# lunarlab-gatech/SLIDE_SLAM

Hardware: AMD Instinct MI355X
Metric: pose-graph updates/sec + ms/Gauss-Newton iter, 8-robot 10k-landmark graph (higher is better)
Workload: dtype f64

## Files before the change

slide_slam_amd/csrc/chol_kernels.hip:

```cpp
#include <hip/hip_runtime.h>
#include <stdlib.h>
#include <algorithm>
#include <type_traits>
#include <utility>
#include <vector>

#include "graph_dev.hpp"
#include "kernels.hpp"

namespace sl {

typedef double v4d __attribute__((ext_vector_type(4)));
constexpr int CHOL_BATCH_MAX = 8;
__device__ inline v4d mfma_f64(double a, double b, v4d c) { return __builtin_amdgcn_mfma_f64_16x16x4f64(a, b, c, 0, 0, 0); }

__device__ inline double rsqrt_nr(double d) {
#ifdef SLIDE_RSQRT_OLD
  double y = __builtin_amdgcn_rsq(d);
  y = y * (1.5 - 0.5 * d * y * y);
  y = y * (1.5 - 0.5 * d * y * y);
  return y;
#else
  double y = __builtin_amdgcn_rsq(d);
  double t = d * y, h = 0.5 * y;
// ... 2551 lines not shown
    const int ka = std::max(1, ks_sys ? ks_sys[0] : ks), kb = std::max(1, ks_sys ? ks_sys[1] : ks), km = std::max(ka, kb);
    A.ks = km; A.scratch = scratch; A.scratch_stride = std::max<size_t>(1, (size_t)(nb + 1) * nb * (km - 1) * NB * NB);
    A.ks_sys[0] = ka; A.ks_sys[1] = kb;
    launch_syrk_kernel(dim3(njobs, 1, km), lds_pad, s, A);
    hipLaunchKernelGGL(k_border_syrk_reduce2, dim3(16 * (nb + 1), jb_end >= 0 ? jb_end : nb), dim3(256), 0, s, d[0].bord, d[0].ldb, d[1].bord, d[1].ldb, nb,
                       ka, kb, scratch, scratch + A.scratch_stride, d[0].T, d[1].T);
    return;
  }
  if (scratch && n == 1 && ks > 1) {
    A.ks = ks; A.scratch = scratch;
    launch_syrk_kernel(dim3(njobs, 1, ks), lds_pad, s, A);
    const int nb = d[0].nbr;
    hipLaunchKernelGGL(k_border_syrk_reduce, dim3(16 * (nb + 1), jb_end >= 0 ? jb_end : nb), dim3(256), 0, s, d[0].bord, d[0].ldb, nb, ks, scratch, d[0].bfirst, d[0].T);
    return;
  }
  launch_syrk_kernel(dim3(njobs), lds_pad, s, A);
}
struct BorderApplyArgs {
  int n;
  const double* S[CHOL_BATCH_MAX]; int ld[CHOL_BATCH_MAX]; int T[CHOL_BATCH_MAX]; int nbr[CHOL_BATCH_MAX]; int b0[CHOL_BATCH_MAX];
  double* yv[CHOL_BATCH_MAX]; const double* x[CHOL_BATCH_MAX];
  const int* segtab[CHOL_BATCH_MAX];
};
__global__ __launch_bounds__(256) void k_border_apply(BorderApplyArgs A) {
  const int r = blockIdx.z;
  const int col = blockIdx.x * 4 + (threadIdx.x >> 6), lane = threadIdx.x & 63;
  if (col >= A.T[r] * NB) return;
  const int nrow = A.nbr[r] * NB;
  const double* w = A.S[r] + (size_t)col * A.ld[r] + (size_t)A.b0[r] * NB;
  const double* x = A.x[r];
  double acc = 0.0;
  const int* st = A.segtab[r];
  const int* msk = st ? st + 1 + st[0] + st[0] * (A.nbr[r] + 1) : nullptr;
  if (msk && msk[0] > 0) {
    const int c = col / NB;
    unsigned long long m = (unsigned long long)(unsigned)msk[1 + 2 * c] | ((unsigned long long)(unsigned)msk[2 + 2 * c] << 32);
    while (m) {
      const int t = __ffsll((long long)m) - 1;
      m &= m - 1;
      acc += w[t * NB + lane] * x[t * NB + lane];
    }
  } else {
    for (int q = lane; q < nrow; q += 64) acc += w[q] * x[q];
  }
#pragma unroll
  for (int m = 32; m >= 1; m >>= 1) acc += __shfl_xor(acc, m);
  if (lane == 0) A.yv[r][col] -= acc;
}
void launch_border_apply(const CholSystem* d, int n, const double* const* xloc, hipStream_t s) {
  BorderApplyArgs A{};
  A.n = n;
  int Tmax = 0;
  for (int i = 0; i < n; ++i) {
    A.S[i] = d[i].S; A.ld[i] = d[i].ld; A.T[i] = d[i].T; A.nbr[i] = d[i].nbr; A.yv[i] = d[i].yv; A.x[i] = xloc[i];
    A.b0[i] = d[i].b0 > 0 ? d[i].b0 : d[i].T;
    A.segtab[i] = d[i].segtab;
    Tmax = d[i].T > Tmax ? d[i].T : Tmax;
  }
  if (Tmax > 0) hipLaunchKernelGGL(k_border_apply, dim3(Tmax * NB / 4, 1, n), dim3(256), 0, s, A);
}

void launch_chol_bwd_all(const double* S, int ld, int T, const double* Ld, const double* Winv, double* yv, double* dp,
                         int* status, const int* prof, hipStream_t s, const double* wf_prev, double wf_thr, int wf_Tprev, int wf_lim);
void launch_chol_extract_y(const double* S, int ld, int T, double* yv, double* dp, int* status, hipStream_t s, int nbr, int b0, double* prev) {
  hipLaunchKernelGGL(k_chol_extract_y, dim3((T * NB + 255) / 256), dim3(256), 0, s, S, ld, T, (b0 > 0 ? b0 : T) + nbr, yv, dp, status, prev);
}
struct StepPlan { int kb, nP, g0, g1, nX, TvA, TvB, TvX, nbA, nbB, nbX; long long nA, nB; };
static int chol_n_cu() {
  static int n_cu = 0;
  if (!n_cu) {
    int dev = 0;
    hipDeviceProp_t pr;
    if (hipGetDevice(&dev) == hipSuccess && hipGetDeviceProperties(&pr, dev) == hipSuccess) n_cu = pr.multiProcessorCount;
    if (n_cu <= 0) n_cu = 256;
  }
  return n_cu;
}
static StepPlan plan_step(int k, int T, const int* prof, int nbr = 0, const int* bfirst = nullptr, int kofs = 0) {
  static const double frac = getenv("SLIDE_CHOL_FRAC") ? atof(getenv("SLIDE_CHOL_FRAC")) : 0.5;
  StepPlan p{};
  p.kb = k & ~1;
  p.TvA = p.TvB = p.TvX = T;
// ... 77 lines not shown
    for (int i = 0; i < n; ++i) {
      const PairPlan p = plan_pair(k, d[i].T, d[i].h_prof, d[i].nbr, d[i].h_bfirst, d[i].kofs);
      A.S[i] = d[i].S; A.ld[i] = d[i].ld; A.Ld[i] = d[i].Ld; A.Winv[i] = d[i].Winv; A.status[i] = d[i].status;
      A.ncols[i] = p.ncols; A.Tv0[i] = p.Tv0; A.Tv1[i] = p.Tv1; A.nb0[i] = p.nb0; A.nb1[i] = p.nb1;
      A.TvB[i] = p.TvB; A.nbB[i] = p.nbB; A.nP[i] = p.nP;
      A.nbr[i] = d[i].nbr; A.B0[i] = d[i].b0 > 0 ? d[i].b0 : d[i].T; A.ord[i] = d[i].ord;
      A.a_base[i + 1] = A.a_base[i] + (int)(2 * p.nA);
      A.b_base[i + 1] = A.b_base[i] + (int)p.nB;
    }
    const long long nAw = A.a_base[n], nB = A.b_base[n];
    if (nAw <= 0) continue;
    const long long extra = nB < n_cu ? nB : n_cu;
    const long long free_cu = n_cu - nAw > 8 ? n_cu - nAw : 8;
    const int a_joins = nB > free_cu ? 1 : 0;
    hipLaunchKernelGGL(k_chol_pair_batched, dim3((unsigned)(nAw + extra)), dim3(PAIR_THREADS), 0, s, A, k, ctr, tickets, a_joins);
  }
}
bool chol_pair_supported(const CholSystem* d, int n) {
  if (n < 1 || n > CHOL_STEP_BATCH_MAX) return false;
  for (int i = 0; i < n; ++i)
    if (d[i].L32) return false;
  return true;
}
void launch_chol_batch(const CholSystem* d, int n, int* ctr, hipStream_t s, hipEvent_t after_steps, bool solve, int cu_share, int* pair_tickets) {
  const bool pair = pair_tickets != nullptr;
  const int n_cu = chol_n_cu();
  int Tmax = 0;
  for (int i = 0; i < n; ++i) Tmax = d[i].T > Tmax ? d[i].T : Tmax;
  static const bool verify = getenv("SLIDE_PAIR_VERIFY") && getenv("SLIDE_PAIR_VERIFY")[0] == '1';
  if (pair && chol_pair_supported(d, n) && verify) {
    (void)hipStreamSynchronize(s);
    std::vector<CholSystem> cp(d, d + n);
    std::vector<size_t> len(n);
    std::vector<void*> tmp;
    auto dmal = [&](size_t bytes) { void* p = nullptr; (void)hipMalloc(&p, bytes); tmp.push_back(p); return p; };
    for (int i = 0; i < n; ++i) {
      const int B0 = d[i].b0 > 0 ? d[i].b0 : d[i].T;
      len[i] = (size_t)d[i].ld * ((size_t)d[i].T * NB - 1) + (size_t)(B0 + d[i].nbr + 1) * NB;
      cp[i].S = (double*)dmal(len[i] * sizeof(double));
      cp[i].Ld = (double*)dmal((size_t)d[i].T * NB * NB * sizeof(double));
      cp[i].Winv = (double*)dmal((size_t)d[i].T * 1024 * sizeof(double));
      cp[i].status = (int*)dmal(8 * sizeof(int));
      cp[i].yv = (double*)dmal((size_t)d[i].T * NB * sizeof(double));
      cp[i].dp = (double*)dmal((size_t)d[i].T * NB * sizeof(double));
      (void)hipMemset(cp[i].status, 0, 8 * sizeof(int));
      (void)hipMemcpy(cp[i].S, d[i].S, len[i] * sizeof(double), hipMemcpyDeviceToDevice);
    }
// ... 43 lines not shown
    const int a_split = (k > 0 && (nA2 + nBt) * 100 <= (long long)n_cu * share) ? 1 : 0;
    A.a_base[0] = A.b_base[0] = 0;
    for (int i = 0; i < n; ++i) {
      A.S[i] = d[i].S; A.ld[i] = d[i].ld; A.T[i] = d[i].T; A.Ld[i] = d[i].Ld; A.Winv[i] = d[i].Winv; A.status[i] = d[i].status;
      A.L32[i] = d[i].L32;
      A.TvA[i] = pl[i].TvA; A.TvB[i] = pl[i].TvB; A.TvX[i] = pl[i].TvX;
      A.nP[i] = pl[i].nP; A.g0[i] = pl[i].g0; A.g1[i] = pl[i].g1; A.nX[i] = pl[i].nX; A.a_split[i] = a_split;
      A.nbr[i] = d[i].nbr; A.nbA[i] = pl[i].nbA; A.nbB[i] = pl[i].nbB; A.nbX[i] = pl[i].nbX;
      A.B0[i] = d[i].b0 > 0 ? d[i].b0 : d[i].T;
      A.ord[i] = d[i].ord;
      A.a_base[i + 1] = A.a_base[i] + (int)(pl[i].nA << a_split);
      A.b_base[i + 1] = A.b_base[i] + (int)pl[i].nB;
    }
    const long long nAw = A.a_base[n], nB = A.b_base[n];
    const long long extra = nB < n_cu ? nB : n_cu;
    const long long free_cu = n_cu - nAw > 8 ? n_cu - nAw : 8;
    const int a_joins = nB > free_cu ? 1 : 0;
    static const int xcd_map = getenv("SLIDE_CHOL_XCD") ? atoi(getenv("SLIDE_CHOL_XCD")) : 0;
    hipLaunchKernelGGL(k_chol_step_batched, dim3((unsigned)(nAw + extra)), dim3(512), 0, s, A, k, k & ~1, ctr, a_joins, (xcd_map && n > 1) ? 1 : 0);
  }
  if (Tmax < 0) Tmax = -Tmax;
  if (after_steps) (void)hipEventRecord(after_steps, s);
  if (!solve) {
    ExtractArgs E{};
    E.n = n;
    for (int i = 0; i < n; ++i) {
      E.S[i] = d[i].S; E.ld[i] = d[i].ld; E.T[i] = d[i].T; E.Tr[i] = (d[i].b0 > 0 ? d[i].b0 : d[i].T) + d[i].nbr;
      E.yv[i] = d[i].yv; E.dp[i] = d[i].dp; E.status[i] = d[i].status;
    }
    if (Tmax > 0) hipLaunchKernelGGL(k_chol_extract_y_b, dim3((Tmax * NB + 255) / 256, n), dim3(256), 0, s, E);
    return;
  }
  launch_chain_tables(d, n, s);
  const double* yin[CHOL_BATCH_MAX];
  double* xout[CHOL_BATCH_MAX];
  for (int i = 0; i < n; ++i) {
    launch_chol_extract_y(d[i].S, d[i].ld, d[i].T, d[i].yv, d[i].dp, d[i].status, s, d[i].nbr);
    yin[i] = d[i].yv; xout[i] = d[i].dp;
  }
  if (chain_has_tables(d, n)) {
    launch_chain_batch(d, n, yin, xout, false, false, true, nullptr, s);
    return;
  }
  launch_chol_bwd_batch(d, n, s);
}
void launch_chol_bwd_batch(const CholSystem* d, int n, hipStream_t s) {
// ... 197 lines not shown
```

slide_slam_amd/csrc/host_graph.hip:

```cpp
#include <chrono>

#include "host_graph.hpp"

#include <algorithm>
#include <cmath>
#include <cstdio>
#include <cstdlib>
#include <map>
#include <unordered_map>

namespace sl {

static inline int lam_ks_cap(int nl) {
  const int tiles = (nl + 1) * nl;
  if (tiles <= 0) return 1;
  return tiles <= 32 ? 16 : std::max(1, std::min(16, 256 / tiles));
}

thread_local std::string g_last_error;
void thread_capture_mode_local() {
  thread_local bool done = false;
  if (done) return;
  hipStreamCaptureMode m = hipStreamCaptureModeThreadLocal;
  (void)hipThreadExchangeStreamCaptureMode(&m);
// ... 1047 lines not shown
  if (whole || part == 0) {
    if (!whole) launch_bcast(d_bufs, n, 12 * ng, master);
    launch_ghost_exchange_batched(d_Gs, n, ng, 1, d_bufs, master);
  }
  return SLIDE_OK;
}
int CholBatch::enqueue_arrow(double* const* d_bufs, int part, hipEvent_t e0, hipEvent_t e1) {
  const bool whole = part < 0;
  if (part == 20) return enqueue_ghost_refresh(d_bufs, part);
  auto mark = [&](int i) { if (prof_ev[0]) (void)hipEventRecord(prof_ev[i], master); };
  const int* maps[CHOL_BATCH_HOST_MAX];
  double* xloc[CHOL_BATCH_HOST_MAX];
  for (int i = 0; i < n; ++i) { maps[i] = graphs[i]->d_sep_map.d; xloc[i] = graphs[i]->d_xloc.d; }
  const int ld_s = (sep_Ts + sep_nl + 1) * NB;
  const SepLayout Y = sep_layout();
  CholSystem lv[2];
  const int sTa = sep_leafT[0], sTL = sTa + sep_leafT[1], sTt = sep_Ts - sTL;
  if (sep_dissected()) sep_leaf_systems(lv);
  const bool owned = !whole && sep_dissected() && sep_owner >= 0;
  const int own = owned ? sep_owner : 0, own_t0 = own ? sTa : 0, own_T = sep_leafT[own];
  CholSystem top{};
  top.S = sepS + (owned ? (size_t)own_t0 * NB * ld_s : 0); top.ld = ld_s; top.T = owned ? own_T : sTL; top.b0 = sTL; top.nbr = sTt + sep_nl;
  top.bord = sepS + (size_t)sTL * NB * ld_s + (size_t)sTL * NB; top.ldb = ld_s;
  if (part == 1) {
    if (!owned) return SLIDE_OK;
    if (sep_leader) launch_sep_unpack(Y, master, sTL, sep_Ts + sep_nl);
    launch_sep_unpack(Y, master, own_t0, own_t0 + own_T);
    if (ll_leaf_own[own]) launch_chol_ll(ll_leaf_own[own], &lv[own], 1, master);
    else launch_chol_batch(&lv[own], 1, sep_ctr2, master, nullptr, false, 100, (chol_pair_mask() & 4) ? pair_tickets(10) : nullptr);
    if (sep_leader) {
      launch_border_syrk_jobs(&top, 1, d_sep_jobs, n_sep_jobs, 0, master, sep_scratch, sep_ks, sTt);
      if (sep_nl > 0) {
        CholSystem sl{};
        sl.S = sepS + (size_t)own_t0 * NB * ld_s; sl.ld = ld_s; sl.T = own_T; sl.b0 = sep_Ts; sl.nbr = sep_nl; sl.bord = sep_bord; sl.ldb = (sep_nl + 1) * NB;
        const int ks = std::max(1, std::min(lam_ks_cap(sep_nl), own_T / 2));
        launch_border_syrk(&sl, 1, master, lam_scratch, ks);
      }
      launch_sep_unpack(Y, master, sTL, sep_Ts + sep_nl, true);
    }
    return SLIDE_OK;
  }
  if (whole || part == 0) {
    launch_status_clear(d_Gs, n, master, sep_status, sep_nl > 0 ? lam_status : nullptr);
    const int rg = enqueue_ghost_refresh(d_bufs, part);
    if (rg != SLIDE_OK) return rg;
    launch_phase0_batched(d_Gs, hG.data(), n, d_bufs, master, false, rb.on() ? d_Rs : nullptr, ol.on() ? d_Os : nullptr);
    launch_phase3_arrow_batched(d_Gs, hG.data(), n, master);
    {
      int nq[CHOL_BATCH_HOST_MAX];
      for (int i = 0; i < n; ++i) nq[i] = graphs[i]->n_sep_poses;
      launch_sep_extract_batched(d_Gs, hG.data(), n, nq, master);
    }
    if (e0) (void)hipEventRecord(e0, master);
    mark(0);
    if (ll_seg) {
      launch_chol_ll(ll_seg, seg_sys.data(), (int)seg_sys.size(), master);
      last_groups = 1;
      if (e1) (void)hipEventRecord(e1, master);
    } else {
      const int rc = factor_all(e1);
      if (rc != SLIDE_OK) return rc;
    }
    mark(1);
    if (n_syrk_jobs > 0) launch_border_syrk_jobs(sys.data(), n, d_syrk_jobs, n_syrk_jobs, syrk_lds_pad, master);
    else launch_border_syrk(sys.data(), n, master);
    mark(6);
    if (!l2_sys.empty()) {
      if (ll_l2) launch_chol_ll(ll_l2, l2_sys.data(), (int)l2_sys.size(), master);
      else launch_chol_batch(l2_sys.data(), (int)l2_sys.size(), d_ctr2, master, nullptr, false, 100, (chol_pair_mask() & 2) ? pair_tickets(8) : nullptr);
      if (n_l2_jobs > 0) launch_border_syrk_jobs(l2_sys.data(), (int)l2_sys.size(), d_l2_jobs, n_l2_jobs, 0, master);
      else launch_border_syrk(l2_sys.data(), (int)l2_sys.size(), master);
    }
    mark(2);
    static const bool env_canon = !(getenv("SLIDE_SEP_CANONICAL") && getenv("SLIDE_SEP_CANONICAL")[0] == '0');
    const bool canon = whole && sep_dissected() && env_canon && n <= 8;
    if (canon) launch_sep_gather(hG.data(), n, maps, Y, false, master, d_sep_tmask, sTL * NB, sep_mask_b, sep_top2, sep_ld2, sep_bord2);
    else launch_sep_gather(hG.data(), n, maps, Y, !whole, master, d_sep_tmask);
    mark(3);
  }
  if (whole || part == 2) {
    if (!whole && !owned) launch_sep_unpack(Y, master);
    if (owned) launch_sep_unpack(Y, master, sTL, sep_Ts + sep_nl);
    if (sep_dissected()) {
      const int TL = sTL, Tt = sTt;
      static const bool env_canon2 = !(getenv("SLIDE_SEP_CANONICAL") && getenv("SLIDE_SEP_CANONICAL")[0] == '0');
      const bool canon2 = whole && env_canon2 && n <= 8;
      if (!owned) {
        if (ll_leaves) launch_chol_ll(ll_leaves, lv, 2, master);
        else launch_chol_batch(lv, 2, sep_ctr2, master, nullptr, false, 100, (chol_pair_mask() & 4) ? pair_tickets(9) : nullptr);
        if (canon2) {
          CholSystem tp2[2] = {top, top};
          for (int hh = 0; hh < 2; ++hh) {
            tp2[hh].S = sepS + (size_t)(hh ? sTa : 0) * NB * ld_s; tp2[hh].T = sep_leafT[hh]; tp2[hh].b0 = sTL;
            if (hh) { tp2[hh].bord = sep_top2; tp2[hh].ldb = sep_ld2; }
          }
          CholSystem sl2[2];
          int ks_lam[2] = {1, 1};
          for (int hh = 0; hh < 2 && sep_nl > 0; ++hh) {
            CholSystem sl{};
            sl.S = sepS + (size_t)(hh ? sTa : 0) * NB * ld_s; sl.ld = ld_s; sl.T = sep_leafT[hh]; sl.b0 = sep_Ts; sl.nbr = sep_nl;
            sl.bord = hh ? sep_bord2 : sep_bord; sl.ldb = (sep_nl + 1) * NB;
            ks_lam[hh] = std::max(1, std::min(lam_ks_cap(sep_nl), sep_leafT[hh] / 2));
            sl2[hh] = sl;
          }
          if (sep_scratch && (sep_nl == 0 || (lam_scratch && d_lam_jobs2))) {
            launch_border_syrk_jobs(tp2, 2, d_sep_jobs2, n_sep_jobs2, 0, master, sep_scratch, sep_ks, Tt, nullptr, true);
            if (sep_nl > 0) launch_border_syrk_jobs(sl2, 2, d_lam_jobs2, n_lam_jobs2, 0, master, lam_scratch, 1, -1, ks_lam, true);
          } else {
            for (int hh = 0; hh < 2; ++hh) {
              launch_border_syrk_jobs(&tp2[hh], 1, d_sep_jobs, n_sep_jobs, 0, master, sep_scratch, sep_ks, Tt);
              if (sep_nl > 0) launch_border_syrk(&sl2[hh], 1, master, lam_scratch, ks_lam[hh]);
            }
            launch_sep_top_add(Y, sTL, sep_top2, sep_ld2, sep_bord2, master);
          }
        } else {
          launch_border_syrk_jobs(&top, 1, d_sep_jobs, n_sep_jobs, 0, master, sep_scratch, sep_ks, Tt);
        }
      }
      if (ll_top) {
        const CholSystem ts = sep_top_system();
        launch_chol_ll(ll_top, &ts, 1, master);
      } else if ((chol_pair_mask() & 8) && d_pair_tickets) {
        const CholSystem ts = sep_top_system();
        launch_chol_batch(&ts, 1, sep_ctr, master, nullptr, false, 100, pair_tickets(11));
      } else {
        double* St = sepS + (size_t)TL * NB * ld_s + (size_t)TL * NB;
        for (int k = 0; k < Tt; ++k)
          launch_chol_step(St, ld_s, k, Tt, sep_Ld + (size_t)(TL + k) * NB * NB, sep_Winv + (size_t)(TL + k) * 1024, sep_status, sep_ctr, nullptr, nullptr, master, sep_nl);
        launch_chol_extract_y(St, ld_s, Tt, sep_yv + (size_t)TL * NB, sep_dp + (size_t)TL * NB, sep_status, master, sep_nl);
      }
    } else if (ll_top) {
      const CholSystem ts = sep_top_system();
      launch_chol_ll(ll_top, &ts, 1, master);
    } else if ((chol_pair_mask() & 8) && d_pair_tickets) {
      const CholSystem ts = sep_top_system();
      launch_chol_batch(&ts, 1, sep_ctr, master, nullptr, false, 100, pair_tickets(11));
    } else {
      for (int k = 0; k < sep_Ts; ++k)
        launch_chol_step(sepS, ld_s, k, sep_Ts, sep_Ld + (size_t)k * NB * NB, sep_Winv + (size_t)k * 1024, sep_status, sep_ctr, nullptr,
                         sep_prof_on ? h_sep_prof.data() : nullptr, master, sep_nl);
      launch_chol_extract_y(sepS, ld_s, sep_Ts, sep_yv, sep_dp, sep_status, master, sep_nl);
    }
    if (sep_nl > 0) {
      CholSystem ss{};
      ss.S = sepS; ss.ld = ld_s; ss.T = sep_Ts; ss.yv = sep_yv; ss.nbr = sep_nl; ss.bord = sep_bord; ss.ldb = (sep_nl + 1) * NB; ss.bfirst = nullptr;
      CholSystem sr = ss;
      static const bool env_canon3 = !(getenv("SLIDE_SEP_CANONICAL") && getenv("SLIDE_SEP_CANONICAL")[0] == '0');
      if (owned || (whole && sep_dissected() && env_canon3 && n <= 8)) { sr.S = sepS + (size_t)sTL * NB * ld_s; sr.T = sTt; sr.b0 = sep_Ts; }
      const int ks = std::max(1, std::min(lam_ks_cap(sep_nl), sr.T / 2));
      launch_border_syrk(&sr, 1, master, lam_scratch, ks);
      launch_lam_prepare(sep_bord, sep_nl, sep_lam, lamS, master);
      const int ld_l = (sep_nl + 1) * NB;
      for (int k = 0; k < sep_nl; ++k)
        launch_chol_step(lamS, ld_l, k, sep_nl, lam_Ld + (size_t)k * NB * NB, lam_Winv + (size_t)k * 1024, lam_status, lam_ctr, nullptr, nullptr, master);
      launch_chol_extract_y(lamS, ld_l, sep_nl, lam_yv, lam_dp, lam_status, master);
      launch_chol_bwd_all(lamS, ld_l, sep_nl, lam_Ld, lam_Winv, lam_yv, lam_dp, lam_status, nullptr, master);
      const double* xl = lam_dp;
      if (!owned) launch_border_apply(&ss, 1, &xl, master);
      else {
        CholSystem ap2[2] = {ss, ss};
        ap2[0].S = sepS + (size_t)own_t0 * NB * ld_s; ap2[0].T = own_T; ap2[0].b0 = sep_Ts; ap2[0].yv = sep_yv + (size_t)own_t0 * NB;
        ap2[1].S = sepS + (size_t)sTL * NB * ld_s; ap2[1].T = sTt; ap2[1].b0 = sep_Ts; ap2[1].yv = sep_yv + (size_t)sTL * NB;
        const double* xl2[2] = {xl, xl};
        launch_border_apply(ap2, 2, xl2, master);
      }
    }
    if (sep_dissected()) {
      double* St = sepS + (size_t)sTL * NB * ld_s + (size_t)sTL * NB;
      launch_chol_bwd_all(St, ld_s, sTt, sep_Ld + (size_t)sTL * NB * NB, sep_Winv + (size_t)sTL * 1024, sep_yv + (size_t)sTL * NB, sep_dp + (size_t)sTL * NB,
                          sep_status, nullptr, master);
      launch_ints_clear(sep_status + 4, 1, master);
      CholSystem ap[2] = {lv[0], lv[1]};
      ap[0].nbr = ap[1].nbr = sTt;
      const double* xt[2] = {sep_dp + (size_t)sTL * NB, sep_dp + (size_t)sTL * NB};
      if (!owned) {
        launch_border_apply(ap, 2, xt, master);
        launch_chol_bwd_batch(lv, 2, master);
      } else {
        launch_border_apply(&ap[own], 1, xt, master);
        launch_chol_bwd_batch(&lv[own], 1, master);
      }
    } else {
      launch_chol_bwd_all(sepS, ld_s, sep_Ts, sep_Ld, sep_Winv, sep_yv, sep_dp, sep_status, sep_prof_on ? d_sep_prof : nullptr, master);
    }
    mark(4);
    launch_sep_xloc(n, maps, sep_m, sep_lam, sep_dp, lam_dp, xloc, master);
    if (!l2_sys.empty()) {
      const double* x2[CHOL_BATCH_HOST_MAX];
      for (size_t i = 0; i < l2_sys.size(); ++i) x2[i] = xloc[l2_graph[i]] + (size_t)hG[l2_graph[i]].nsep * NB;
      launch_border_apply(l2_sys.data(), (int)l2_sys.size(), x2, master);
      launch_chol_bwd_batch(l2_sys.data(), (int)l2_sys.size(), master);
      launch_ints_clear(l2_sys[0].status + 4, 1, master);
      {
        const double* src[CHOL_BATCH_HOST_MAX]; double* dst[CHOL_BATCH_HOST_MAX]; int cnt[CHOL_BATCH_HOST_MAX];
        for (size_t i = 0; i < l2_sys.size(); ++i) { src[i] = l2_sys[i].dp; dst[i] = xloc[l2_graph[i]]; cnt[i] = hG[l2_graph[i]].nsep * NB; }
        launch_copy_pairs(src, dst, cnt, (int)l2_sys.size(), master);
      }
    }
    launch_border_apply(sys.data(), n, xloc, master);
    launch_chol_bwd_batch(seg_sys.data(), (int)seg_sys.size(), master);
    launch_sep_pose_scatter_batched(d_Gs, hG.data(), n, xloc, master);
    bool slots_onto = true;
    for (int i = 0; i < n; ++i) slots_onto = slots_onto && graphs[i]->lm_slot_onto;
    launch_arrow_finish_batched(d_Gs, hG.data(), n, sep_dp, d_sep_off, master, slots_onto);
    launch_status_gather(d_Gs, n, d_status_all, master, sep_status, sep_nl > 0 ? lam_status : nullptr);
    mark(5);
  }
  return SLIDE_OK;
}
int CholBatch::profile_arrow(double* const* d_bufs, double* out6, int* n_sep_steps) {
  std::lock_guard<std::mutex> pl(pass_mtx);
  exact_serial = 0;
  bool same = false;
  int rc = begin_pass(d_bufs, &same);
  if (rc != SLIDE_OK) return rc;
  if (!(arrow && hG[0].n_slots > 0)) { g_last_error = "profile_arrow: the batch does not run exact joint passes"; return SLIDE_ERR_INVALID; }
  hipEvent_t start = nullptr;
  SL_HIP(hipEventCreate(&start));
  for (auto& e : prof_ev) SL_HIP(hipEventCreate(&e));
  (void)hipEventRecord(start, master);
  rc = enqueue_arrow(d_bufs, -1, nullptr, nullptr);
  const hipError_t es = hipStreamSynchronize(master);
// ... 207 lines not shown
}
void CholBatch::note_pass() {
  rb_pass_done = true;
  lin_rb_kind = rb.kind; lin_rb_mask = rb.mask;
  lin_bt.resize(n); lin_gh.resize(n);
  for (int i = 0; i < n; ++i) { lin_bt[i] = (size_t)graphs[i]->G.n_between; lin_gh[i] = (size_t)graphs[i]->G.n_ghost; }
  ol_pass_done = true;
  lin_ol_kind = ol.kind;
  lin_lf.resize(n);
  for (int i = 0; i < n; ++i) lin_lf[i] = (size_t)graphs[i]->G.n_lf;
}
int CholBatch::end_pass() {
  int st[CHOL_BATCH_HOST_MAX][8];
  SL_HIP(hipMemcpyAsync(st, d_status_all, (size_t)n * 8 * sizeof(int), hipMemcpyDeviceToHost, master));
  SL_HIP(hipStreamSynchronize(master));
  SL_HIP(hipGetLastError());
  for (int i = 0; i < n; ++i) {
    const int rc = decode_status(st[i]);
    if (rc != SLIDE_OK) return rc;
  }
  return SLIDE_OK;
}

int CholBatch::factor_all(hipEvent_t after) {
  static const int env_groups = getenv("SLIDE_CHOL_GROUPS") ? atoi(getenv("SLIDE_CHOL_GROUPS")) : 0;
  const bool exact = arrow && hG[0].n_slots > 0;
  const std::vector<CholSystem>& S_ = exact ? seg_sys : sys;
  const int ns = (int)S_.size();
  bool narrow = true;
  for (int i = 0; i < n; ++i) narrow = narrow && hG[i].schur_split == 1;
  int groups = env_groups > 0 ? env_groups : (narrow ? 4 : 2);
  if (env_groups <= 0 && exact && ns > n) groups = std::max(2, (ns + 11) / 12);
  if (groups > (env_groups > 0 ? ns : ns / 2)) groups = env_groups > 0 ? ns : ns / 2;
  while (groups > 0 && (ns + groups - 1) / groups > CHOL_STEP_BATCH_MAX) ++groups;
  if (groups > 8) groups = 8;
  last_groups = groups < 1 ? 1 : groups;
  const bool solve = !exact;
  if (groups < 2) {
    launch_chol_batch(S_.data(), ns, d_ctr, master, nullptr, solve, 100, (exact && (chol_pair_mask() & 1)) ? pair_tickets(0) : nullptr);
    if (after) SL_HIP(hipEventRecord(after, master));
    return SLIDE_OK;
  }
  if (!ev_aux0) SL_HIP(hipEventCreateWithFlags(&ev_aux0, hipEventDisableTiming));
  SL_HIP(hipEventRecord(ev_aux0, master));
  const int per = (ns + groups - 1) / groups;
  for (int g = 0; g < groups; ++g) {
    const int lo = g * per, hi = std::min(ns, lo + per);
    if (lo >= hi) break;
    hipStream_t st = master;
    if (g > 0) {
      if (!aux[g]) {
        SL_HIP(hipStreamCreateWithFlags(&aux[g], hipStreamNonBlocking));
        SL_HIP(hipEventCreateWithFlags(&ev_aux1[g], hipEventDisableTiming));
      }
      st = aux[g];
      SL_HIP(hipStreamWaitEvent(st, ev_aux0, 0));
    }
    launch_chol_batch(S_.data() + lo, hi - lo, d_ctr + (size_t)g * (ctr_cap / CHOL_BATCH_HOST_MAX), st, nullptr, solve, std::max(25, 100 / groups),
                      (exact && (chol_pair_mask() & 1)) ? pair_tickets(g) : nullptr);
    if (g > 0) {
      SL_HIP(hipEventRecord(ev_aux1[g], st));
      SL_HIP(hipStreamWaitEvent(master, ev_aux1[g], 0));
    }
  }
  if (after) SL_HIP(hipEventRecord(after, master));
  return SLIDE_OK;
}

void CholBatch::set_pcg(int iters, double tol) {
  std::lock_guard<std::mutex> pl(pass_mtx);
  exact_serial = 0;
  std::vector<HostGraph*> gs;
  {
    std::lock_guard<std::mutex> lk(mtx);
    pcg_iters = iters < 0 ? 0 : iters;
    pcg_tol = tol > 0.0 ? tol : 0.0;
    pass_dirty = true;
    gs.assign(graphs.begin(), graphs.end());
  }
  for (HostGraph* g : gs)
    if (g) { std::lock_guard<std::mutex> gl(g->mtx); g->topo_dirty = true; }
}
// ... 1343 lines not shown
```

slide_slam_amd/csrc/host_graph.hpp:

```cpp
#pragma once
#include <hip/hip_runtime.h>

#include <cstdint>
#include <cstring>
#include <condition_variable>
#include <functional>
#include <mutex>
#include <string>
#include <unordered_map>
#include <vector>

#include "../../include/slide_gpu.h"
#include "graph_dev.hpp"
#include "kernels.hpp"
#include "sl_math.hpp"

namespace sl {

extern thread_local std::string g_last_error;
void thread_capture_mode_local();
bool hip_ok(hipError_t e, const char* what);
inline bool robot_ok(int r) { return r >= 0 && r < SLIDE_MAX_ROBOTS; }
int decode_status(const int* st8);
struct LossSetting {
// ... 264 lines not shown
  std::vector<ObsLossDev> hO, pass_O;
  ObsLossDev member_obs_view(const HostGraph* g) const;
  bool ol_pass_done = false;
  int lin_ol_kind = 0;
  std::vector<size_t> lin_lf;
  double* d_ol_out = nullptr; size_t ol_out_cap = 0;
  int capture_pass(double* const* d_bufs, int part, hipGraphExec_t* exec);
  int prepare_pass();
  int prepare_member(HostGraph* g, bool for_pass);
  int begin_pass(double* const* d_bufs, bool* same);
  int end_pass();
  int enqueue_pass(double* const* d_bufs, hipEvent_t e0, hipEvent_t e1, int part);
  std::vector<GraphDev> hG;
  int rendezvous(int slot, hipStream_t s, bool reduce, int count);
  std::vector<hipEvent_t> ev_in;
  hipEvent_t ev_out = nullptr;
  hipStream_t master = nullptr;
  hipStream_t aux[8] = {};
  hipEvent_t ev_aux0 = nullptr, ev_aux1[8] = {};
  int* d_ctr = nullptr;
  int last_groups = 1;
  int* d_status_all = nullptr;
  int ctr_cap = 0;
  int factor_all(hipEvent_t after);
  unsigned long long n_exact = 0, exact_serial = 0, jsig_serial = 0;
  std::vector<std::vector<size_t>> exact_shape;
  double* jsig_sep = nullptr; long long jsig_lds_sep = 0;
  std::vector<double*> jsig_rob; std::vector<long long> jsig_lds;
  std::vector<int*> jsig_prow;
  void free_joint_sigma();
  int joint_state(const char* who, int slot);
  int ensure_joint_sigma();
  GainFetched ig_host;
  int compute_joint_sigma();
  struct JointTree {
    std::vector<JSinvSys> Y;
    std::vector<int> rp{0}, rows;
    std::vector<std::vector<std::vector<int>>> steps;
    std::vector<std::vector<std::pair<int, int>>> ranges;
    std::vector<int> T, Tc, Trow, gn;
    std::vector<std::vector<int>> map, prow;
    int Ts = 0, Tsep = 0, sTa = 0, sTL = 0;
    struct SolvePlan {
      struct Launch { int kind, bwd, j0, nj, maxl; };
      std::vector<Launch> launches;
      std::vector<int4> jobs;
      std::vector<int> lst, sptr{0};
// ... 272 lines not shown
```

slide_slam_amd/csrc/kernels.hpp:

```cpp
#pragma once
#include <hip/hip_runtime.h>
#include <stdint.h>

#include "graph_dev.hpp"
#include "sl_math.hpp"

namespace sl {

void init_solver_kernels();
void launch_relin(const GraphDev& G, hipStream_t s);
void launch_linearize(const GraphDev& G, const ObsLossDev& O, hipStream_t s);
void launch_observation_weights(const GraphDev& G, const ObsLossDev& O, bool robust, int n, double* out2n, hipStream_t s);
void launch_observation_weights_batched(const GraphDev* d, const ObsLossDev* dO, bool robust, const int* off, const int* cnt, int n, double* out2n,
                                        hipStream_t s);
void launch_robust_reweight(const GraphDev& G, const RobustDev& R, hipStream_t s);
void launch_closure_weights(const GraphDev& G, const RobustDev& R, const int* idx, int n, double* out2n, hipStream_t s);
void launch_robust_reweight_batched(const GraphDev* d, const RobustDev* dR, const GraphDev* h, int n, hipStream_t s);
void launch_closure_weights_batched(const GraphDev* d, const RobustDev* dR, const int* ent2, int n, double* out2n, hipStream_t s);
void launch_landmark(const GraphDev& G, int mode, hipStream_t s);
void launch_pose(const GraphDev& G, hipStream_t s);
void launch_schur(const GraphDev& G, hipStream_t s);
void launch_backsub(const GraphDev& G, int mode, hipStream_t s);
void launch_shared_pack(const GraphDev& G, int what, double* buf, hipStream_t s);
void launch_shared_unpack(const GraphDev& G, int what, const double* buf, hipStream_t s);
// ... 10 lines not shown
void launch_phase0_batched(const GraphDev* d, const GraphDev* h, int n, double* const* bufs, hipStream_t s, bool pack = true, const RobustDev* dR = nullptr,
                           const ObsLossDev* dO = nullptr);
void launch_linearize_batched(const GraphDev* d, const GraphDev* h, int n, hipStream_t s, const ObsLossDev* dO = nullptr);
void launch_phase4_batched(const GraphDev* d, const GraphDev* h, int n, double* const* bufs, hipStream_t s);
void launch_phase2_batched(const GraphDev* d, const GraphDev* h, int n, double* const* bufs, hipStream_t s);
void launch_phase3_batched(const GraphDev* d, const GraphDev* h, int n, double* const* bufs, hipStream_t s);
void launch_ghost_exchange(const GraphDev& G, int what, double* buf, hipStream_t s);
void launch_ghost_exchange_batched(const GraphDev* d, int n, int n_gslots, int what, double* const* bufs, hipStream_t s);
void launch_border_assemble_batched(const GraphDev* d, const GraphDev* h, int n, hipStream_t s, bool clear = true, bool fills = true);
void launch_sep_extract_batched(const GraphDev* d, const GraphDev* h, int n, const int* n_sep_poses, hipStream_t s);
void launch_sep_pose_scatter_batched(const GraphDev* d, const GraphDev* h, int n, double* const* xloc, hipStream_t s);
struct SepLayout { double* sys; double* bord; double* packed; int Ts, nl, ms, lam; int gap[4]; int hTa, hTL; };
void launch_ghost_refresh_local(const GraphDev* d, int n, int n_gslots, hipStream_t s);
void launch_copy_pairs(const double* const* src, double* const* dst, const int* count, int n, hipStream_t s);
void launch_sep_gather(const GraphDev* h, int n, const int* const* maps, const SepLayout& Y, bool packed, hipStream_t s, const int* tmask = nullptr,
                       int split_col = -1, unsigned mask_b = 0, double* sys2 = nullptr, int ld2 = 0, double* bord2 = nullptr);
void launch_sep_top_add(const SepLayout& Y, int c0, const double* sys2, int ld2, const double* bord2, hipStream_t s);
void launch_sep_unpack(const SepLayout& Y, hipStream_t s, int c0 = 0, int c1 = -1, bool to_packed = false);
void launch_lam_prepare(const double* bord, int nl, int lam, double* out, hipStream_t s);
void launch_sep_xloc(int n, const int* const* maps, int ms, int lam, const double* xs, const double* xl, double* const* xloc, hipStream_t s);
void launch_arrow_finish_batched(const GraphDev* d, const GraphDev* h, int n, const double* xs, const int* sep_off, hipStream_t s, bool slots_onto);
struct AsmMerge { int mask; };
AsmMerge asm_merge_env();
void launch_phase3_arrow_batched(const GraphDev* d, const GraphDev* h, int n, hipStream_t s);

void launch_chol_step(double* S, int ld, int k, int T, double* Ld, double* Winv, int* status, int* ctr, float* L32, const int* h_prof, hipStream_t s, int nbr = 0);
void launch_chol_extract_y(const double* S, int ld, int T, double* yv, double* dp, int* status, hipStream_t s, int nbr = 0, int b0 = 0, double* prev = nullptr);
constexpr unsigned long long CHAIN_SENTINEL = 0x7FF8DEADBEEF0BADull;
struct CholSystem { double* S; int ld, T; double* Ld; double* Winv; double* yv; double* dp; int* status;
                    float* L32;
                    const int* h_prof;
                    const int* prof; const int* first;
                    double* ctab;
                    int nbr;
                    double* bord; int ldb;
                    const double* bord_src;
                    const int* bfirst;
                    const int* h_bfirst;
                    int b0;
                    int kofs;
                    const int* ord;
                    const int* segtab; };
constexpr int CHOL_STEP_BATCH_MAX = 32;
void launch_chol_batch(const CholSystem* d, int n, int* ctr, hipStream_t s, hipEvent_t after_steps = nullptr, bool solve = true, int cu_share = 100, int* pair_tickets = nullptr);
bool chol_pair_supported(const CholSystem* d, int n);
void launch_chol_bwd_batch(const CholSystem* d, int n, hipStream_t s);
struct CholLLPlan;
CholLLPlan* chol_ll_plan_create(const CholSystem* d, int n, const int* const* h_ord = nullptr, hipStream_t upload_stream = nullptr);
void chol_ll_plan_destroy(CholLLPlan* p);
int chol_ll_plan_tasks(const CholLLPlan* p);
int chol_ll_plan_columns(const CholLLPlan* p);
void launch_chol_ll(const CholLLPlan* p, const CholSystem* d, int n, hipStream_t s, int* trace = nullptr);
void launch_border_syrk(const CholSystem* d, int n, hipStream_t s, double* scratch = nullptr, int ks = 1);
void launch_border_syrk_jobs(const CholSystem* d, int n, const int* jobs, int njobs, int lds_pad, hipStream_t s, double* scratch = nullptr, int ks = 1, int jb_end = -1,
                             const int* ks_sys = nullptr, bool fuse_add = false);
void launch_border_apply(const CholSystem* d, int n, const double* const* xloc, hipStream_t s);
void launch_chain_batch(const CholSystem* d, int n, const double* const* in, double* const* out, bool fwd, bool f32, bool prepared,
                        double* const* next_out, hipStream_t s);
void launch_chain_tables(const CholSystem* d, int n, hipStream_t s);
void launch_chol_bwd_all(const double* S, int ld, int T, const double* Ld, const double* Winv, double* yv, double* dp, int* status, const int* prof, hipStream_t s,
                         const double* wf_prev = nullptr, double wf_thr = 0.0, int wf_Tprev = 0, int wf_lim = -1);
void launch_pose_covariance(const double* S, int ld, int T, const double* Ld, const double* Winv, double* Y, int row0, double* cov36,
                            hipStream_t s);
void launch_selected_inverse(const double* S, int ld, int T, const double* Ld, const double* Winv, const int* prof, const int* d_prof,
                             double* Sg, double* Z, hipStream_t s);
void launch_pose_blocks(const double* Sg, int ld, const int* poses, int n, double* out, hipStream_t s, const int* prow = nullptr);
void launch_landmark_covariances(const GraphDev& G, const double* Sg, int ld, const int* lids, int n, double* out, hipStream_t s,
                                 const int* prow = nullptr);
void launch_multi_solve(const double* S, int ld, int T, const double* Ld, const double* Winv, const int* prof, double* B, double* X,
                        int nrhs, hipStream_t s);
void launch_multi_fwd(const double* S, int ld, int T, const double* Ld, const double* Winv, const int* prof, double* B, double* W,
                      int nrhs, hipStream_t s, int k0 = 0);
void launch_gram(const double* X, size_t ldx, int ncol, const int* rows, int nrows, double* M, hipStream_t s);
void launch_landmark_V(const GraphDev& G, const double* U, int nT, int ncol, const int* lids, int n, double* V, size_t ldv, hipStream_t s,
                       const int* prow = nullptr);
void launch_scatter(const int* rc, const double* val, int n, double* B, int nT, hipStream_t s);
constexpr int GAIN_MAX_STEPS = 64, GAIN_MAX_GRAMS = 4, GAIN_LDS_DIM = 96;
struct GainCandDev { int c0, nk, nsplit, pad; long long moff, poff, woff; };
int gain_gram_splits(int nk);
// ... 203 lines not shown
```

slide_slam_amd/csrc/solver_kernels.hip:

```cpp
#include <hip/hip_runtime.h>
#include <algorithm>
#include <cstring>

#include "graph_dev.hpp"
#include "kernels.hpp"
#include "sl_math.hpp"

namespace sl {

struct BufPtrs { double* p[8]; };

__device__ inline void pose_retract12(const double* in12, const double* d6, int chart, double* out12) {
  to12(retract(from12(in12), d6, chart), out12);
}
__device__ inline void lm_retract(int type, const double* in, const double* d, int chart, double* out) {
  if (type == VT_POINT) {
    out[0] = in[0] + d[0]; out[1] = in[1] + d[1]; out[2] = in[2] + d[2];
  } else if (type == VT_CUBE) {
    pose_retract12(in, d, chart, out);
    out[12] = in[12] + d[6]; out[13] = in[13] + d[7]; out[14] = in[14] + d[8];
  } else {
    out[3] = in[3] + d[0]; out[4] = in[4] + d[1]; out[5] = in[5] + d[2];
    out[0] = in[0] + d[3]; out[1] = in[1] + d[4]; out[2] = in[2] + d[5];
    out[6] = in[6] + d[6];
// ... 1620 lines not shown
  if (t >= 12 * G.n_gslots) return;
  if (what == 0) {
    const int p = G.gslot_pose[t / 12];
    buf[t] = p >= 0 ? G.pose_est[12 * (size_t)p + t % 12] : 0.0;
  } else {
    G.ghost_val[t] = buf[t];
  }
}
__global__ void k_ghost_refresh_local(const GraphDev* __restrict__ Gs, int n) {
  const GraphDev G = Gs[blockIdx.z];
  const int t = blockIdx.x * blockDim.x + threadIdx.x;
  if (t >= 12 * G.n_gslots) return;
  double v = 0.0;
  for (int q = 0; q < n; ++q) {
    const int p = Gs[q].gslot_pose[t / 12];
    v += p >= 0 ? Gs[q].pose_est[12 * (size_t)p + t % 12] : 0.0;
  }
  G.ghost_val[t] = v;
}
void launch_ghost_refresh_local(const GraphDev* d, int n, int n_gslots, hipStream_t s) {
  if (n_gslots <= 0 || n <= 0) return;
  hipLaunchKernelGGL(k_ghost_refresh_local, dim3((12 * n_gslots + 127) / 128, 1, n), dim3(128), 0, s, d, n);
}
void launch_ghost_exchange_batched(const GraphDev* d, int n, int n_gslots, int what, double* const* bufs, hipStream_t s) {
  if (n_gslots <= 0 || n <= 0) return;
  GhostBufs B{};
  for (int i = 0; i < n; ++i) B.p[i] = bufs[i];
  hipLaunchKernelGGL(k_ghost_exchange_b, dim3((12 * n_gslots + 127) / 128, 1, n), dim3(128), 0, s, d, what, B);
}

__device__ __forceinline__ void k_estimate_body(const GraphDev& G) {
  const int t = blockIdx.x * blockDim.x + threadIdx.x;
  if (t < G.P) {
    pose_retract12(G.pose_val + 12 * (size_t)t, G.pose_delta + 6 * (size_t)t, G.chart, G.pose_est + 12 * (size_t)t);
  } else if (t < G.P + G.L) {
    const int l = t - G.P;
    lm_retract(G.lm_type[l], G.lm_val + 15 * (size_t)l, G.lm_delta + 9 * (size_t)l, G.chart, G.lm_est + 15 * (size_t)l);
  }
}
__global__ void k_estimate(GraphDev G) { k_estimate_body(G); }
__global__ void k_estimate_predict(GraphDev G, int pose, double* __restrict__ out) {
  k_estimate_body(G);
  const int t = blockIdx.x * blockDim.x + threadIdx.x;
  int dirty = 0;
  if (t < G.P) {
    double mx = 0.0;
// ... 521 lines not shown
```

Baseline: 4138.

## Fold y-extraction and ticket reset into border-apply kernel across solve passes

```diff
diff --git a/slide_slam_amd/csrc/chol_kernels.hip b/slide_slam_amd/csrc/chol_kernels.hip
--- a/slide_slam_amd/csrc/chol_kernels.hip
+++ b/slide_slam_amd/csrc/chol_kernels.hip
@@ -2597,14 +2597,24 @@
   double* yv[CHOL_BATCH_MAX]; const double* x[CHOL_BATCH_MAX];
   const int* segtab[CHOL_BATCH_MAX];
 };
-__global__ __launch_bounds__(256) void k_border_apply(BorderApplyArgs A) {
+struct BorderPrepArgs { BorderApplyPrep p[CHOL_BATCH_MAX]; };
+template <bool PREP>
+__device__ __forceinline__ void border_apply_body(const BorderApplyArgs& A, const BorderPrepArgs* Pp) {
   const int r = blockIdx.z;
+  if (PREP && blockIdx.x == 0 && threadIdx.x == 0 && Pp->p[r].ticket) *Pp->p[r].ticket = 0;
   const int col = blockIdx.x * 4 + (threadIdx.x >> 6), lane = threadIdx.x & 63;
   if (col >= A.T[r] * NB) return;
   const int nrow = A.nbr[r] * NB;
   const double* w = A.S[r] + (size_t)col * A.ld[r] + (size_t)A.b0[r] * NB;
   const double* x = A.x[r];
   double acc = 0.0;
+  bool prep = false;
+  double rhs = 0.0;
+  if (PREP && lane == 0) {
+    const BorderApplyPrep& P = Pp->p[r];
+    for (int k = 0; k < P.n_ranges; ++k) prep = prep || (col / NB >= P.lo[k] && col / NB < P.hi[k]);
+    if (prep) rhs = A.S[r][(size_t)col * A.ld[r] + (size_t)P.rhs_row * NB];
+  }
   const int* st = A.segtab[r];
   const int* msk = st ? st + 1 + st[0] + st[0] * (A.nbr[r] + 1) : nullptr;
   if (msk && msk[0] > 0) {
@@ -2620,9 +2630,17 @@
   }
 #pragma unroll
   for (int m = 32; m >= 1; m >>= 1) acc += __shfl_xor(acc, m);
-  if (lane == 0) A.yv[r][col] -= acc;
-}
-void launch_border_apply(const CholSystem* d, int n, const double* const* xloc, hipStream_t s) {
+  if (lane != 0) return;
+  if (PREP && prep) {
+    A.yv[r][col] = rhs - acc;
+    Pp->p[r].dp[col] = __longlong_as_double((long long)BWD_SENT);
+    return;
+  }
+  A.yv[r][col] -= acc;
+}
+__global__ __launch_bounds__(256) void k_border_apply(BorderApplyArgs A) { border_apply_body<false>(A, nullptr); }
+__global__ __launch_bounds__(256) void k_border_apply_prep(BorderApplyArgs A, BorderPrepArgs P) { border_apply_body<true>(A, &P); }
+void launch_border_apply(const CholSystem* d, int n, const double* const* xloc, hipStream_t s, const BorderApplyPrep* prep) {
   BorderApplyArgs A{};
   A.n = n;
   int Tmax = 0;
@@ -2632,7 +2650,11 @@
     A.segtab[i] = d[i].segtab;
     Tmax = d[i].T > Tmax ? d[i].T : Tmax;
   }
-  if (Tmax > 0) hipLaunchKernelGGL(k_border_apply, dim3(Tmax * NB / 4, 1, n), dim3(256), 0, s, A);
+  if (Tmax <= 0) return;
+  if (!prep) { hipLaunchKernelGGL(k_border_apply, dim3(Tmax * NB / 4, 1, n), dim3(256), 0, s, A); return; }
+  BorderPrepArgs P{};
+  for (int i = 0; i < n; ++i) P.p[i] = prep[i];
+  hipLaunchKernelGGL(k_border_apply_prep, dim3(Tmax * NB / 4, 1, n), dim3(256), 0, s, A, P);
 }
 
 void launch_chol_bwd_all(const double* S, int ld, int T, const double* Ld, const double* Winv, double* yv, double* dp,
@@ -2756,7 +2778,7 @@
     if (d[i].L32) return false;
   return true;
 }
-void launch_chol_batch(const CholSystem* d, int n, int* ctr, hipStream_t s, hipEvent_t after_steps, bool solve, int cu_share, int* pair_tickets) {
+void launch_chol_batch(const CholSystem* d, int n, int* ctr, hipStream_t s, hipEvent_t after_steps, bool solve, int cu_share, int* pair_tickets, bool extract) {
   const bool pair = pair_tickets != nullptr;
   const int n_cu = chol_n_cu();
   int Tmax = 0;
@@ -2846,6 +2868,7 @@
   if (Tmax < 0) Tmax = -Tmax;
   if (after_steps) (void)hipEventRecord(after_steps, s);
   if (!solve) {
+    if (!extract) return;
     ExtractArgs E{};
     E.n = n;
     for (int i = 0; i < n; ++i) {
diff --git a/slide_slam_amd/csrc/host_graph.hip b/slide_slam_amd/csrc/host_graph.hip
--- a/slide_slam_amd/csrc/host_graph.hip
+++ b/slide_slam_amd/csrc/host_graph.hip
@@ -1093,6 +1093,21 @@
   CholSystem top{};
   top.S = sepS + (owned ? (size_t)own_t0 * NB * ld_s : 0); top.ld = ld_s; top.T = owned ? own_T : sTL; top.b0 = sTL; top.nbr = sTt + sep_nl;
   top.bord = sepS + (size_t)sTL * NB * ld_s + (size_t)sTL * NB; top.ldb = ld_s;
+  const int fold = pass_fold_env().mask;
+  const bool fold_sep = (fold & 1) && !owned;
+  const bool top_fold = fold_sep && sep_nl > 0 && !ll_top;
+  const bool leaf_fold = fold_sep && sep_dissected() && !ll_leaves && (sep_nl == 0 || top_fold);
+  const bool l2_fold = (fold & 1) && !l2_sys.empty() && !ll_l2;
+  bool rob_fold = (fold & 1) && !ll_seg;
+  for (int i = 0; i < n; ++i) rob_fold = rob_fold && graphs[i]->segs.size() <= 8;
+  std::vector<CholSystem> l2v(l2_sys);
+  const bool xl_fold = (fold & 2) && !l2_sys.empty() && !ll_l2;
+  if (xl_fold) for (size_t i = 0; i < l2v.size(); ++i) l2v[i].dp = xloc[l2_graph[i]];
+  auto prep_all = [](const CholSystem& c, bool extract) {
+    BorderApplyPrep p{};
+    p.n_ranges = extract ? 1 : 0; p.lo[0] = 0; p.hi[0] = c.T; p.rhs_row = (c.b0 > 0 ? c.b0 : c.T) + c.nbr; p.dp = c.dp; p.ticket = c.status + 4;
+    return p;
+  };
   if (part == 1) {
     if (!owned) return SLIDE_OK;
     if (sep_leader) launch_sep_unpack(Y, master, sTL, sep_Ts + sep_nl);
@@ -1129,7 +1144,7 @@
       last_groups = 1;
       if (e1) (void)hipEventRecord(e1, master);
     } else {
-      const int rc = factor_all(e1);
+      const int rc = factor_all(e1, !rob_fold);
       if (rc != SLIDE_OK) return rc;
     }
     mark(1);
@@ -1138,7 +1153,7 @@
     mark(6);
     if (!l2_sys.empty()) {
       if (ll_l2) launch_chol_ll(ll_l2, l2_sys.data(), (int)l2_sys.size(), master);
-      else launch_chol_batch(l2_sys.data(), (int)l2_sys.size(), d_ctr2, master, nullptr, false, 100, (chol_pair_mask() & 2) ? pair_tickets(8) : nullptr);
+      else launch_chol_batch(l2v.data(), (int)l2v.size(), d_ctr2, master, nullptr, false, 100, (chol_pair_mask() & 2) ? pair_tickets(8) : nullptr, !l2_fold);
       if (n_l2_jobs > 0) launch_border_syrk_jobs(l2_sys.data(), (int)l2_sys.size(), d_l2_jobs, n_l2_jobs, 0, master);
       else launch_border_syrk(l2_sys.data(), (int)l2_sys.size(), master);
     }
@@ -1158,7 +1173,7 @@
       const bool canon2 = whole && env_canon2 && n <= 8;
       if (!owned) {
         if (ll_leaves) launch_chol_ll(ll_leaves, lv, 2, master);
-        else launch_chol_batch(lv, 2, sep_ctr2, master, nullptr, false, 100, (chol_pair_mask() & 4) ? pair_tickets(9) : nullptr);
+        else launch_chol_batch(lv, 2, sep_ctr2, master, nullptr, false, 100, (chol_pair_mask() & 4) ? pair_tickets(9) : nullptr, !leaf_fold);
         if (canon2) {
           CholSystem tp2[2] = {top, top};
           for (int hh = 0; hh < 2; ++hh) {
@@ -1193,24 +1208,24 @@
         launch_chol_ll(ll_top, &ts, 1, master);
       } else if ((chol_pair_mask() & 8) && d_pair_tickets) {
         const CholSystem ts = sep_top_system();
-        launch_chol_batch(&ts, 1, sep_ctr, master, nullptr, false, 100, pair_tickets(11));
+        launch_chol_batch(&ts, 1, sep_ctr, master, nullptr, false, 100, pair_tickets(11), !top_fold);
       } else {
         double* St = sepS + (size_t)TL * NB * ld_s + (size_t)TL * NB;
         for (int k = 0; k < Tt; ++k)
           launch_chol_step(St, ld_s, k, Tt, sep_Ld + (size_t)(TL + k) * NB * NB, sep_Winv + (size_t)(TL + k) * 1024, sep_status, sep_ctr, nullptr, nullptr, master, sep_nl);
-        launch_chol_extract_y(St, ld_s, Tt, sep_yv + (size_t)TL * NB, sep_dp + (size_t)TL * NB, sep_status, master, sep_nl);
+        if (!top_fold) launch_chol_extract_y(St, ld_s, Tt, sep_yv + (size_t)TL * NB, sep_dp + (size_t)TL * NB, sep_status, master, sep_nl);
       }
     } else if (ll_top) {
       const CholSystem ts = sep_top_system();
       launch_chol_ll(ll_top, &ts, 1, master);
     } else if ((chol_pair_mask() & 8) && d_pair_tickets) {
       const CholSystem ts = sep_top_system();
-      launch_chol_batch(&ts, 1, sep_ctr, master, nullptr, false, 100, pair_tickets(11));
+      launch_chol_batch(&ts, 1, sep_ctr, master, nullptr, false, 100, pair_tickets(11), !top_fold);
     } else {
       for (int k = 0; k < sep_Ts; ++k)
         launch_chol_step(sepS, ld_s, k, sep_Ts, sep_Ld + (size_t)k * NB * NB, sep_Winv + (size_t)k * 1024, sep_status, sep_ctr, nullptr,
                          sep_prof_on ? h_sep_prof.data() : nullptr, master, sep_nl);
-      launch_chol_extract_y(sepS, ld_s, sep_Ts, sep_yv, sep_dp, sep_status, master, sep_nl);
+      if (!top_fold) launch_chol_extract_y(sepS, ld_s, sep_Ts, sep_yv, sep_dp, sep_status, master, sep_nl);
     }
     if (sep_nl > 0) {
       CholSystem ss{};
@@ -1227,8 +1242,11 @@
       launch_chol_extract_y(lamS, ld_l, sep_nl, lam_yv, lam_dp, lam_status, master);
       launch_chol_bwd_all(lamS, ld_l, sep_nl, lam_Ld, lam_Winv, lam_yv, lam_dp, lam_status, nullptr, master);
       const double* xl = lam_dp;
-      if (!owned) launch_border_apply(&ss, 1, &xl, master);
-      else {
+      if (!owned) {
+        BorderApplyPrep ps{};
+        ps.n_ranges = 1; ps.lo[0] = 0; ps.hi[0] = sep_Ts; ps.rhs_row = sep_Ts + sep_nl; ps.dp = sep_dp; ps.ticket = sep_status + 4;
+        launch_border_apply(&ss, 1, &xl, master, top_fold ? &ps : nullptr);
+      } else {
         CholSystem ap2[2] = {ss, ss};
         ap2[0].S = sepS + (size_t)own_t0 * NB * ld_s; ap2[0].T = own_T; ap2[0].b0 = sep_Ts; ap2[0].yv = sep_yv + (size_t)own_t0 * NB;
         ap2[1].S = sepS + (size_t)sTL * NB * ld_s; ap2[1].T = sTt; ap2[1].b0 = sep_Ts; ap2[1].yv = sep_yv + (size_t)sTL * NB;
@@ -1240,12 +1258,13 @@
       double* St = sepS + (size_t)sTL * NB * ld_s + (size_t)sTL * NB;
       launch_chol_bwd_all(St, ld_s, sTt, sep_Ld + (size_t)sTL * NB * NB, sep_Winv + (size_t)sTL * 1024, sep_yv + (size_t)sTL * NB, sep_dp + (size_t)sTL * NB,
                           sep_status, nullptr, master);
-      launch_ints_clear(sep_status + 4, 1, master);
+      if (!fold_sep) launch_ints_clear(sep_status + 4, 1, master);
       CholSystem ap[2] = {lv[0], lv[1]};
       ap[0].nbr = ap[1].nbr = sTt;
       const double* xt[2] = {sep_dp + (size_t)sTL * NB, sep_dp + (size_t)sTL * NB};
       if (!owned) {
-        launch_border_apply(ap, 2, xt, master);
+        const BorderApplyPrep pl[2] = {prep_all(lv[0], leaf_fold && sep_nl == 0), prep_all(lv[1], leaf_fold && sep_nl == 0)};
+        launch_border_apply(ap, 2, xt, master, fold_sep ? pl : nullptr);
         launch_chol_bwd_batch(lv, 2, master);
       } else {
         launch_border_apply(&ap[own], 1, xt, master);
@@ -1259,16 +1278,27 @@
     if (!l2_sys.empty()) {
       const double* x2[CHOL_BATCH_HOST_MAX];
       for (size_t i = 0; i < l2_sys.size(); ++i) x2[i] = xloc[l2_graph[i]] + (size_t)hG[l2_graph[i]].nsep * NB;
-      launch_border_apply(l2_sys.data(), (int)l2_sys.size(), x2, master);
-      launch_chol_bwd_batch(l2_sys.data(), (int)l2_sys.size(), master);
-      launch_ints_clear(l2_sys[0].status + 4, 1, master);
-      {
+      BorderApplyPrep p2[CHOL_BATCH_HOST_MAX];
+      for (size_t i = 0; i < l2v.size(); ++i) p2[i] = prep_all(l2v[i], true);
+      launch_border_apply(l2v.data(), (int)l2v.size(), x2, master, l2_fold ? p2 : nullptr);
+      launch_chol_bwd_batch(l2v.data(), (int)l2v.size(), master);
+      if (!rob_fold) launch_ints_clear(l2_sys[0].status + 4, 1, master);
+      if (!xl_fold) {
         const double* src[CHOL_BATCH_HOST_MAX]; double* dst[CHOL_BATCH_HOST_MAX]; int cnt[CHOL_BATCH_HOST_MAX];
         for (size_t i = 0; i < l2_sys.size(); ++i) { src[i] = l2_sys[i].dp; dst[i] = xloc[l2_graph[i]]; cnt[i] = hG[l2_graph[i]].nsep * NB; }
         launch_copy_pairs(src, dst, cnt, (int)l2_sys.size(), master);
       }
     }
-    launch_border_apply(sys.data(), n, xloc, master);
+    BorderApplyPrep pr[CHOL_BATCH_HOST_MAX];
+    for (int i = 0; i < n && rob_fold; ++i) {
+      pr[i] = prep_all(sys[i], true);
+      const std::vector<HostGraph::Seg>& sg = graphs[i]->segs;
+      if (hG[i].nsep > 0 && !sg.empty()) {
+        pr[i].n_ranges = (int)sg.size();
+        for (size_t k = 0; k < sg.size(); ++k) { pr[i].lo[k] = sg[k].t0; pr[i].hi[k] = sg[k].t1; }
+      }
+    }
+    launch_border_apply(sys.data(), n, xloc, master, rob_fold ? pr : nullptr);
     launch_chol_bwd_batch(seg_sys.data(), (int)seg_sys.size(), master);
     launch_sep_pose_scatter_batched(d_Gs, hG.data(), n, xloc, master);
     bool slots_onto = true;
@@ -1522,7 +1552,7 @@
   return SLIDE_OK;
 }
 
-int CholBatch::factor_all(hipEvent_t after) {
+int CholBatch::factor_all(hipEvent_t after, bool extract) {
   static const int env_groups = getenv("SLIDE_CHOL_GROUPS") ? atoi(getenv("SLIDE_CHOL_GROUPS")) : 0;
   const bool exact = arrow && hG[0].n_slots > 0;
   const std::vector<CholSystem>& S_ = exact ? seg_sys : sys;
@@ -1537,7 +1567,7 @@
   last_groups = groups < 1 ? 1 : groups;
   const bool solve = !exact;
   if (groups < 2) {
-    launch_chol_batch(S_.data(), ns, d_ctr, master, nullptr, solve, 100, (exact && (chol_pair_mask() & 1)) ? pair_tickets(0) : nullptr);
+    launch_chol_batch(S_.data(), ns, d_ctr, master, nullptr, solve, 100, (exact && (chol_pair_mask() & 1)) ? pair_tickets(0) : nullptr, extract);
     if (after) SL_HIP(hipEventRecord(after, master));
     return SLIDE_OK;
   }
@@ -1557,7 +1587,7 @@
       SL_HIP(hipStreamWaitEvent(st, ev_aux0, 0));
     }
     launch_chol_batch(S_.data() + lo, hi - lo, d_ctr + (size_t)g * (ctr_cap / CHOL_BATCH_HOST_MAX), st, nullptr, solve, std::max(25, 100 / groups),
-                      (exact && (chol_pair_mask() & 1)) ? pair_tickets(g) : nullptr);
+                      (exact && (chol_pair_mask() & 1)) ? pair_tickets(g) : nullptr, extract);
     if (g > 0) {
       SL_HIP(hipEventRecord(ev_aux1[g], st));
       SL_HIP(hipStreamWaitEvent(master, ev_aux1[g], 0));
diff --git a/slide_slam_amd/csrc/host_graph.hpp b/slide_slam_amd/csrc/host_graph.hpp
--- a/slide_slam_amd/csrc/host_graph.hpp
+++ b/slide_slam_amd/csrc/host_graph.hpp
@@ -310,7 +310,7 @@
   int last_groups = 1;
   int* d_status_all = nullptr;
   int ctr_cap = 0;
-  int factor_all(hipEvent_t after);
+  int factor_all(hipEvent_t after, bool extract = true);
   unsigned long long n_exact = 0, exact_serial = 0, jsig_serial = 0;
   std::vector<std::vector<size_t>> exact_shape;
   double* jsig_sep = nullptr; long long jsig_lds_sep = 0;
diff --git a/slide_slam_amd/csrc/kernels.hpp b/slide_slam_amd/csrc/kernels.hpp
--- a/slide_slam_amd/csrc/kernels.hpp
+++ b/slide_slam_amd/csrc/kernels.hpp
@@ -56,6 +56,8 @@
 void launch_arrow_finish_batched(const GraphDev* d, const GraphDev* h, int n, const double* xs, const int* sep_off, hipStream_t s, bool slots_onto);
 struct AsmMerge { int mask; };
 AsmMerge asm_merge_env();
+struct PassFold { int mask; };
+PassFold pass_fold_env();
 void launch_phase3_arrow_batched(const GraphDev* d, const GraphDev* h, int n, hipStream_t s);
 
 void launch_chol_step(double* S, int ld, int k, int T, double* Ld, double* Winv, int* status, int* ctr, float* L32, const int* h_prof, hipStream_t s, int nbr = 0);
@@ -76,7 +78,7 @@
                     const int* ord;
                     const int* segtab; };
 constexpr int CHOL_STEP_BATCH_MAX = 32;
-void launch_chol_batch(const CholSystem* d, int n, int* ctr, hipStream_t s, hipEvent_t after_steps = nullptr, bool solve = true, int cu_share = 100, int* pair_tickets = nullptr);
+void launch_chol_batch(const CholSystem* d, int n, int* ctr, hipStream_t s, hipEvent_t after_steps = nullptr, bool solve = true, int cu_share = 100, int* pair_tickets = nullptr, bool extract = true);
 bool chol_pair_supported(const CholSystem* d, int n);
 void launch_chol_bwd_batch(const CholSystem* d, int n, hipStream_t s);
 struct CholLLPlan;
@@ -88,7 +90,8 @@
 void launch_border_syrk(const CholSystem* d, int n, hipStream_t s, double* scratch = nullptr, int ks = 1);
 void launch_border_syrk_jobs(const CholSystem* d, int n, const int* jobs, int njobs, int lds_pad, hipStream_t s, double* scratch = nullptr, int ks = 1, int jb_end = -1,
                              const int* ks_sys = nullptr, bool fuse_add = false);
-void launch_border_apply(const CholSystem* d, int n, const double* const* xloc, hipStream_t s);
+struct BorderApplyPrep { int n_ranges; int lo[8], hi[8]; int rhs_row; double* dp; int* ticket; };
+void launch_border_apply(const CholSystem* d, int n, const double* const* xloc, hipStream_t s, const BorderApplyPrep* prep = nullptr);
 void launch_chain_batch(const CholSystem* d, int n, const double* const* in, double* const* out, bool fwd, bool f32, bool prepared,
                         double* const* next_out, hipStream_t s);
 void launch_chain_tables(const CholSystem* d, int n, hipStream_t s);
diff --git a/slide_slam_amd/csrc/solver_kernels.hip b/slide_slam_amd/csrc/solver_kernels.hip
--- a/slide_slam_amd/csrc/solver_kernels.hip
+++ b/slide_slam_amd/csrc/solver_kernels.hip
@@ -1666,6 +1666,11 @@
   if (n_gslots <= 0 || n <= 0) return;
   hipLaunchKernelGGL(k_ghost_refresh_local, dim3((12 * n_gslots + 127) / 128, 1, n), dim3(128), 0, s, d, n);
 }
+PassFold pass_fold_env() {
+  PassFold F{3};
+  if (const char* e = getenv("SLIDE_PASS_FOLD")) F.mask = atoi(e);
+  return F;
+}
 void launch_ghost_exchange_batched(const GraphDev* d, int n, int n_gslots, int what, double* const* bufs, hipStream_t s) {
   if (n_gslots <= 0 || n <= 0) return;
   GhostBufs B{};
```

Measured after the change: 4163 (median of 6 runs). Within noise of the previous version (+0.6%).
